# Celebrandil/CudaSift

Hardware: AMD Instinct MI355X
Metric: 1920x1080 SIFT frames/sec (higher is better)
Workload: dtype f32

## Files before the change

### cudasift_amd/csrc/kernels_dog.hip

```cpp
#include <stdlib.h>
#include <string.h>
#include <math.h>
#include "common.hpp"
#include "chain.hpp"

#define WAVES_PER_BLOCK 4
#define OUT_LANES 62

struct ItemCoord { int frame, strip, seg; bool valid; };

__device__ __forceinline__ ItemCoord decode_item(const StripGeom &g)
{
  const unsigned lb = (g.noremap & 1) ? blockIdx.x : xcd_remap(blockIdx.x, gridDim.x);
  const int wave = __builtin_amdgcn_readfirstlane((int)(threadIdx.x >> 6));
  const long long item = (long long)lb * WAVES_PER_BLOCK + wave;
  const long long nitems = (long long)g.nframes * g.nstrips * g.nsegs;
  ItemCoord c;
  c.valid = item < nitems;
  if (g.noremap & 2) {
    c.strip = (int)(item % g.nstrips);
    const long long r = item / g.nstrips;
    c.seg = (int)(r % g.nsegs);
    c.frame = (int)(r / g.nsegs);
  } else {
// ... 878 lines not shown
    if (threadIdx.x == 0) STAMP_MAX(14);
    if (threadIdx.x == 0 && lb + 1 == gridDim.x) STAMP_MAX(16);
    if (threadIdx.x == 0 && lb == (unsigned)nchain) STAMP_MAX(17);
#endif
    if (lb < (unsigned)nchain) {
      const int tiles = C.tiles_x * C.tiles_y;
#if SCAN_RING
      float *chain_lds = reinterpret_cast<float *>(&s_win[0][0]);
#else
      float *chain_lds = s_chain_lds;
#endif
      scaledown_chain_block(const_cast<float *>(scratch), C, k5, (int)(lb % tiles), (int)(lb / tiles), chain_lds);
      asm volatile("s_waitcnt vmcnt(0)" ::: "memory");
      __builtin_amdgcn_fence(__ATOMIC_RELEASE, "workgroup");
      __syncthreads();
      STAMP_MAX(9);
      if (threadIdx.x == 0) {
        unsigned *spare = counters + (size_t)G.nframes * CNT_STRIDE;
        const unsigned sub = lb & 15u, members = ((unsigned)nchain - sub + 15u) / 16u;
        if (atomicAdd(&spare[64 + 32 * sub], 1u) == members - 1u) {
          const unsigned nsub = (unsigned)nchain < 16u ? (unsigned)nchain : 16u;
          if (atomicAdd(&spare[32], 1u) == nsub - 1u && G.wait_ticks != 0u) {
            __hip_atomic_fetch_or(&spare[0], 0x80000000u, __ATOMIC_RELAXED, __HIP_MEMORY_SCOPE_AGENT);
            STAMP_MAX(18);
          }
        }
      }
      STAMP_MAX(19);
      return;
    }
    lb -= (unsigned)nchain;
    if (G.wait_lev < G.nlev && (long long)lb * WAVES_PER_BLOCK + (WAVES_PER_BLOCK - 1) >= G.o[G.wait_lev].item_begin) {
      STAMP_MAX(15);
      __shared__ unsigned s_chain_ok;
      if (threadIdx.x == 0) {
        const unsigned long long t0 = wall_clock64();
        unsigned ok = 1u;
        while ((__hip_atomic_fetch_add(&counters[(size_t)G.nframes * CNT_STRIDE], 1u, __ATOMIC_RELAXED, __HIP_MEMORY_SCOPE_AGENT) &
                0x80000000u) == 0u) {
          if (wall_clock64() - t0 > (unsigned long long)G.wait_ticks) { ok = 0u; break; }
          __builtin_amdgcn_s_sleep(8);
        }
        if (!ok) atomicAdd(&counters[CNT_CHAINTMO], 1u);
        s_chain_ok = ok;
      }
      __syncthreads();
      STAMP_MAX(13);
      __builtin_amdgcn_fence(__ATOMIC_ACQUIRE, "workgroup");
      chain_failed = s_chain_ok == 0u;
    }
  }
  long long item = (long long)lb * WAVES_PER_BLOCK + wave;
  const bool valid = item < G.total_items && !chain_failed;
  __shared__ unsigned s_cq[WAVES_PER_BLOCK][CQ_CAP];
  unsigned qn = 0;
  unsigned *cnt = nullptr, *list = nullptr;
  unsigned cand_cap = 0;
  int octave = 0;
  bool stamp_coarse = false;
  (void)stamp_coarse;
  if (valid) {
    int lev = 0;
    for (int k = 1; k < G.nlev; k++)
      if (item >= G.o[k].item_begin) lev = k;
    lev = __builtin_amdgcn_readfirstlane(lev);
    stamp_coarse = lev >= G.wait_lev;
    const ScanOct &L = G.o[lev];
    item -= L.item_begin;
    const int seg = (int)(item % L.nsegs);
    const long long r = item / L.nsegs;
    const int strip = (int)(r % L.nstrips);
    const int frame = (int)(r / L.nstrips);
    if (lane < NUM_SCAN_PAIRS * 5) s_taps[wave][lane] = scan_pair_tap(taps.t[L.octave], lane);
    wave_lds_fence();
    const int q = strip * (OUT_LANES - 2) + lane - 2;
    const int y0 = seg * L.seg_rows;
    cnt = counters + (size_t)frame * CNT_STRIDE;
    list = cand + (size_t)frame * G.cand_stride + L.cand_off;
    cand_cap = L.cand_cap;
    octave = L.octave;
#if SCAN_TAPS_REG
    const RegTaps tsrc(s_taps[wave]);
#else
    const LdsTaps tsrc{s_taps[wave]};
#endif
#if SCAN_RING
    scan_strip_ring<FAST>(scratch + (long long)frame * G.frame_stride + L.img_off, L.w, L.h, L.p, q, lane, y0,
                          min(y0 + L.seg_rows, L.h), tsrc, thresh, cnt, list, cand_cap, octave, FAST != 0,
                          &s_win[wave][lane], s_cq[wave], qn, xch);
#else
    scan_strip<FAST>(scratch + (long long)frame * G.frame_stride + L.img_off, L.w, L.h, L.p, q, lane, y0,
                     min(y0 + L.seg_rows, L.h), tsrc, thresh, cnt, list, cand_cap, octave, FAST != 0,
                     s_cq[wave], qn, xch);
#endif
  }
#if SCAN_STAMPS
  if (CHAIN && valid) { if (stamp_coarse) STAMP_MAX(12); else STAMP_MAX(11); }
#endif
  scan_queue_finish(s_cq[wave], qn, valid ? cnt + CNT_CAND + octave : nullptr, cnt, list, cand_cap);
}

struct RefineParams {
  int width, height, pitch, nframes;
  float edge_limit, factor, lowest_scale, subsampling, thresh;
  float scmul[NUM_SCALES];
  int octave, max_pts;
  unsigned cand_cap;
};

__device__ __forceinline__ void dog_patch(const float *img, int w, int h, int pitch, const float (&tk)[4][5],
                                          int x, int y, float (&d)[3][3][3])
{
  int xo[11];
#pragma unroll
  for (int cx = 0; cx < 11; cx++) xo[cx] = clampi(x + cx - 5, 0, w - 1);
  float prev[3][3];
#pragma unroll
  for (int bs = 0; bs < 4; bs++) {
    const float k0 = tk[bs][0], k1 = tk[bs][1], k2 = tk[bs][2], k3 = tk[bs][3], k4 = tk[bs][4];
    float vres[3][11];
#pragma unroll
    for (int cx = 0; cx < 11; cx++) {
      const float *col = img + xo[cx];
      float r[11];
#pragma unroll
      for (int j = 0; j < 11; j++) r[j] = col[(size_t)clampi(y + j - 5, 0, h - 1) * pitch];
#pragma unroll
      for (int dy = 0; dy < 3; dy++)
        vres[dy][cx] = conv9(k0, k1, k2, k3, k4, r[dy + 4], r[dy + 3] + r[dy + 5], r[dy + 2] + r[dy + 6],
                             r[dy + 1] + r[dy + 7], r[dy + 0] + r[dy + 8]);
    }
#pragma unroll
    for (int dy = 0; dy < 3; dy++)
#pragma unroll
      for (int dx = 0; dx < 3; dx++) {
        const float *v = &vres[dy][dx];
        const float cur = conv9(k0, k1, k2, k3, k4, v[4], v[3] + v[5], v[2] + v[6], v[1] + v[7], v[0] + v[8]);
        if (bs > 0) d[bs - 1][dy][dx] = cur - prev[dy][dx];
        prev[dy][dx] = cur;
      }
  }
}

__device__ __forceinline__ float det_exp2(float x)
{
  const bool tiny = x < -125.0f;
  x = x > 126.0f ? 126.0f : x;
  x = tiny ? 0.0f : x;
  const float n = rintf(x);
  const float r = x - n;
  float p = __builtin_fmaf(1.535336188319500e-4f, r, 1.339887440266574e-3f);
  p = __builtin_fmaf(p, r, 9.618437357674640e-3f);
  p = __builtin_fmaf(p, r, 5.550332471162809e-2f);
  p = __builtin_fmaf(p, r, 2.402264791363012e-1f);
  p = __builtin_fmaf(p, r, 6.931472028550421e-1f);
  p = __builtin_fmaf(p, r, 1.0f);
  const float sc = __builtin_bit_cast(float, ((int)n + 127) << 23);
  return tiny ? 0.0f : p * sc;
}

struct Refined { float xpos, ypos, scale, sharpness, edgeness; };
__device__ __forceinline__ bool refine_math(const float (&d)[3][3][3], int x, int y, int s, float thresh,
                                            float edge_limit, float factor, float lowest_scale,
                                            const float (&scmul)[NUM_SCALES], Refined &out, bool *extremum = nullptr)
{
  const float val = d[1][1][1];
  if (extremum) *extremum = false;
  {
    float minv = INFINITY, maxv = -INFINITY;
#pragma unroll
    for (int p = 0; p < 3; p++)
#pragma unroll
      for (int dy = 0; dy < 3; dy++)
#pragma unroll
        for (int dx = 0; dx < 3; dx++)
          if (!(p == 1 && dy == 1 && dx == 1)) {
            minv = fminf(minv, d[p][dy][dx]);
            maxv = fmaxf(maxv, d[p][dy][dx]);
          }
    if (!((val < fminf(-thresh, minv)) || (val > fmaxf(thresh, maxv)))) return false;
    if (extremum) *extremum = true;
  }
  const float dxx = 2.0f * val - d[1][1][0] - d[1][1][2];
  const float dyy = 2.0f * val - d[1][0][1] - d[1][2][1];
  const float dxy = 0.25f * (d[1][2][2] + d[1][0][0] - d[1][0][2] - d[1][2][0]);
  const float tra = dxx + dyy;
  const float det = dxx * dyy - dxy * dxy;
  if (!(tra * tra < edge_limit * det)) return false;
  const float edge = (tra * tra) / det;
  const float dx = 0.5f * (d[1][1][2] - d[1][1][0]);
  const float dy = 0.5f * (d[1][2][1] - d[1][0][1]);
  const float ds = 0.5f * (d[0][1][1] - d[2][1][1]);
  const float dss = 2.0f * val - d[2][1][1] - d[0][1][1];
  const float dxs = 0.25f * (d[2][1][2] + d[0][1][0] - d[0][1][2] - d[2][1][0]);
  const float dys = 0.25f * (d[2][2][1] + d[0][0][1] - d[2][0][1] - d[0][2][1]);
  const float idxx = dyy * dss - dys * dys;
  const float idxy = dys * dxs - dxy * dss;
  const float idxs = dxy * dys - dyy * dxs;
  const float idet = 1.0f / (idxx * dxx + idxy * dxy + idxs * dxs);
  const float idyy = dxx * dss - dxs * dxs;
  const float idys = dxy * dxs - dxx * dys;
  const float idss = dxx * dyy - dxy * dxy;
  float pdx = idet * (idxx * dx + idxy * dy + idxs * ds);
  float pdy = idet * (idxy * dx + idyy * dy + idys * ds);
  float pds = idet * (idxs * dx + idys * dy + idss * ds);
  if (pdx < -0.5f || pdx > 0.5f || pdy < -0.5f || pdy > 0.5f || pds < -0.5f || pds > 0.5f) {
    pdx = dx / dxx;
    pdy = dy / dyy;
    pds = ds / dss;
  }
  const float dval = 0.5f * (dx * pdx + dy * pdy + ds * pds);
  float scm = scmul[0];
#pragma unroll
  for (int j = 1; j < NUM_SCALES; j++) scm = (s == j) ? scmul[j] : scm;
  const float sc = scm * det_exp2(pds * factor);
  if (!(sc >= lowest_scale)) return false;
  out.xpos = x + pdx;
  out.ypos = y + pdy;
  out.scale = sc;
  out.sharpness = val + dval;
  out.edgeness = edge;
  return true;
}

__device__ __forceinline__ void dog_from_base(const float *img, int w, int h, int pitch, const LaplaceTaps &taps,
                                              int x, int y, int s, float (&d)[3][3][3])
{
  float tk[4][5];
#pragma unroll
  for (int bs = 0; bs < 4; bs++)
#pragma unroll
    for (int j = 0; j < 5; j++) {
      float t = taps.k[bs][j];
#pragma unroll
      for (int ss = 1; ss < NUM_SCALES; ss++) t = (s == ss) ? taps.k[ss + bs][j] : t;
      tk[bs][j] = t;
    }
  dog_patch(img, w, h, pitch, tk, x, y, d);
}

template <bool FROM_BASE>
__global__ __launch_bounds__(64) void refine_kernel(const float *__restrict__ src, long long src_frame_stride,
                                                    LaplaceTaps taps, RefineParams P,
                                                    unsigned *__restrict__ counters,
                                                    const unsigned *__restrict__ cand, SiftPointD *__restrict__ pts)
{
  const int frame = blockIdx.y;
  unsigned *cnt = counters + (size_t)frame * CNT_STRIDE;
  const unsigned *list = cand + (size_t)frame * P.cand_cap;
  SiftPointD *out = pts + (size_t)frame * P.max_pts;
  const float *img = src + (long long)frame * src_frame_stride;
  const int o = P.octave;
  if (blockIdx.x == 0 && threadIdx.x == 0) {
    const unsigned start = cnt[2 * o - 1];
    atomicMax(&cnt[2 * o + 0], start);
    atomicMax(&cnt[2 * o + 1], start);
  }
  const unsigned ncand = min(cnt[CNT_CAND + o], P.cand_cap);
  const size_t plane = (size_t)P.height * P.pitch;
  for (unsigned ci = blockIdx.x * blockDim.x + threadIdx.x; ci < ncand; ci += gridDim.x * blockDim.x) {
    const unsigned code = list[ci];
    if (code == 0xffffffffu) continue;
    const int x = code & 0x3fff, y = (code >> 14) & 0x3fff, s = code >> 28;
    float d[3][3][3];
    if (FROM_BASE) {
      dog_from_base(img, P.width, P.height, P.pitch, taps, x, y, s, d);
    } else {
#pragma unroll
      for (int p = 0; p < 3; p++)
#pragma unroll
        for (int dy = 0; dy < 3; dy++)
#pragma unroll
          for (int dx = 0; dx < 3; dx++)
            d[p][dy][dx] = img[(size_t)(s + p) * plane + (size_t)(y + dy - 1) * P.pitch + (x + dx - 1)];
    }
    Refined r;
    if (!refine_math(d, x, y, s, P.thresh, P.edge_limit, P.factor, P.lowest_scale, P.scmul, r)) continue;
    atomicMax(&cnt[2 * o + 0], cnt[2 * o - 1]);
    const unsigned idx = atomicAdd(&cnt[2 * o + 0], 1u);
    if (idx >= (unsigned)P.max_pts) { atomicAdd(&cnt[CNT_PTOVF], 1u); continue; }
    SiftPointD *p = &out[idx];
    p->xpos = r.xpos;
    p->ypos = r.ypos;
    p->scale = r.scale;
    p->sharpness = r.sharpness;
    p->edgeness = r.edgeness;
    p->subsampling = P.subsampling;
  }
}

#define REFCAP_W 30
#define REFCAP_H 8
#define REFCAP_WORDS 8
struct RefineAllParams {
  float thresh, edge_limit, factor;
  float scmul[NUM_SCALES];
  int max_pts;
  unsigned cand_stride;
  unsigned cap_words;
  unsigned cap_limit;
  unsigned cap_off[MISIFT_MAX_OCTAVES + 1];
  int cap_tx[MISIFT_MAX_OCTAVES + 1], cap_ty[MISIFT_MAX_OCTAVES + 1];
};
template <int CTRL>
__device__ __forceinline__ float row_dpp(float v)
{
  return __builtin_bit_cast(float, __builtin_amdgcn_mov_dpp(__builtin_bit_cast(int, v), CTRL, 0xf, 0xf, true));
}
#define ROW_SHR(n) (0x110 + (n))
#define ROW_SHL(n) (0x100 + (n))

__global__ __launch_bounds__(256) void refine_all_kernel(const float *__restrict__ scratch, PyramidInfo P,
                                                         AllTaps taps, RefineAllParams R,
                                                         unsigned *__restrict__ counters,
                                                         const unsigned *__restrict__ cand,
                                                         Detection *__restrict__ det, unsigned *__restrict__ capcnt)
{
  const int frame = blockIdx.y;
  unsigned *cnt = counters + (size_t)frame * CNT_STRIDE;
  Detection *fdet = det + (size_t)frame * MISIFT_MAX_OCTAVES * R.max_pts;
  const int lane = threadIdx.x & 63, c = lane & 15;
  const unsigned group = (blockIdx.x * 4u + (threadIdx.x >> 6)) * 4u + (unsigned)(lane >> 4);
  const unsigned ngroups = gridDim.x * 16u;
  unsigned ncand[MISIFT_MAX_OCTAVES + 1];
  unsigned total = 0;
#pragma unroll
  for (int k = 1; k <= MISIFT_MAX_OCTAVES; k++) {
    ncand[k] = k <= P.noct ? __builtin_amdgcn_readfirstlane(min(cnt[CNT_CAND + k], P.o[k].cand_cap)) : 0u;
    total += ncand[k];
  }
  __shared__ unsigned s_n[MISIFT_MAX_OCTAVES + 1], s_base[MISIFT_MAX_OCTAVES + 1];
  if (threadIdx.x <= MISIFT_MAX_OCTAVES) s_n[threadIdx.x] = 0;
  __syncthreads();
  const unsigned rounds = (total + ngroups - 1) / ngroups;
  for (unsigned it = 0; it < rounds; it++) {
    const unsigned fi = it * ngroups + group;
    const bool live = fi < total;
    int o = P.noct;
    unsigned ci = live ? fi : 0u;
    bool found = false;
#pragma unroll
    for (int k = MISIFT_MAX_OCTAVES; k >= 1; k--) {
      if (!found && k <= P.noct) {
        if (ci < ncand[k]) { o = k; found = true; }
        else ci -= ncand[k];
      }
    }
    const int lw = P.o[o].w, lh = P.o[o].h, lp = P.o[o].p;
    const float *img = scratch + (long long)frame * P.frame_stride + P.o[o].img_off;
    const unsigned code = live ? cand[(size_t)frame * R.cand_stride + P.o[o].cand_off + ci] : 0u;
    const int x = code & 0x3fff, y = (code >> 14) & 0x3fff, s = code >> 28;
    const float *col = img + clampi(x + min(c, 10) - 5, 0, lw - 1);
    float r[11];
#pragma unroll
    for (int j = 0; j < 11; j++) r[j] = col[(size_t)clampi(y + j - 5, 0, lh - 1) * lp];
    float ps[3][4];
#pragma unroll
    for (int dy = 0; dy < 3; dy++)
#pragma unroll
      for (int k = 1; k <= 4; k++) ps[dy][k - 1] = r[dy + 4 - k] + r[dy + 4 + k];
    float d[3][3];
    float prev[3];
#pragma unroll
    for (int bs = 0; bs < 4; bs++) {
      const float *tk = taps.t[o].k[s + bs];
      const float k0 = tk[0], k1 = tk[1], k2 = tk[2], k3 = tk[3], k4 = tk[4];
#pragma unroll
      for (int dy = 0; dy < 3; dy++) {
        const float v = conv9(k0, k1, k2, k3, k4, r[dy + 4], ps[dy][0], ps[dy][1], ps[dy][2], ps[dy][3]);
        const float cur = conv9(k0, k1, k2, k3, k4, v,
                                row_dpp<ROW_SHR(1)>(v) + row_dpp<ROW_SHL(1)>(v),
                                row_dpp<ROW_SHR(2)>(v) + row_dpp<ROW_SHL(2)>(v),
                                row_dpp<ROW_SHR(3)>(v) + row_dpp<ROW_SHL(3)>(v),
                                row_dpp<ROW_SHR(4)>(v) + row_dpp<ROW_SHL(4)>(v));
        if (bs > 0) d[bs - 1][dy] = cur - prev[dy];
        prev[dy] = cur;
      }
    }
    float dd[3][3][3];
#pragma unroll
    for (int p = 0; p < 3; p++)
#pragma unroll
      for (int dy = 0; dy < 3; dy++) {
        dd[p][dy][0] = row_dpp<ROW_SHR(1)>(d[p][dy]);
        dd[p][dy][1] = d[p][dy];
        dd[p][dy][2] = row_dpp<ROW_SHL(1)>(d[p][dy]);
      }
    Refined rr;
    bool extremum = false;
    const bool ok = live && c == 5 &&
                    refine_math(dd, x, y, s, R.thresh, R.edge_limit, R.factor, P.o[o].lowest_scale, R.scmul, rr, &extremum);
    if (R.cap_words && live && c == 5 && extremum) {
      const unsigned idx = R.cap_off[o] + ((unsigned)s * R.cap_ty[o] + (unsigned)(y / REFCAP_H)) * R.cap_tx[o] + (unsigned)(x / REFCAP_W);
      const unsigned sh = 8u * (idx & 3u);
      const unsigned old = atomicAdd(&capcnt[(size_t)frame * R.cap_words + (idx >> 2)], 1u << sh);
      if (((old >> sh) & 0xffu) == R.cap_limit) atomicAdd(&cnt[CNT_CANDOVF], 1u);
    }
    unsigned rank = 0;
    if (ok) rank = atomicAdd(&s_n[o], 1u);
    __syncthreads();
    if (threadIdx.x >= 1 && threadIdx.x <= MISIFT_MAX_OCTAVES) {
      const unsigned n = s_n[threadIdx.x];
      if (n) {
        s_base[threadIdx.x] = atomicAdd(&cnt[CNT_DET + threadIdx.x], n);
        s_n[threadIdx.x] = 0;
      }
    }
    __syncthreads();
    if (!ok) continue;
    const unsigned idx = s_base[o] + rank;
    if (idx >= (unsigned)R.max_pts) { atomicAdd(&cnt[CNT_PTOVF], 1u); continue; }
    Detection *pd = &fdet[(size_t)(o - 1) * R.max_pts + idx];
    pd->xpos = rr.xpos;
    pd->ypos = rr.ypos;
    pd->scale = rr.scale;
    pd->sharpness = rr.sharpness;
    pd->edgeness = rr.edgeness;
  }
}

static inline bool is_aligned16(const void *p, int pitch) { return (((uintptr_t)p) & 15) == 0 && (pitch & 3) == 0; }

static inline dim3 grid_for(const StripGeom &g)
{
  const long long nitems = (long long)g.nframes * g.nstrips * g.nsegs;
  return dim3((unsigned)((nitems + WAVES_PER_BLOCK - 1) / WAVES_PER_BLOCK));
}

int launch_laplace(misift_ctx *ctx, const float *base, const StripGeom &g, float *dog,
                   long long dog_frame_stride, const LaplaceTaps &taps)
{
  const int al = is_aligned16(base, g.pitch) && is_aligned16(dog, g.pitch) && (g.frame_stride & 3) == 0 &&
                 (dog_frame_stride & 3) == 0;
  LaunchScope ls(ctx, "laplace");
  if (al && (g.width & 3) == 0)
    hipLaunchKernelGGL(laplace_kernel<true>, grid_for(g), dim3(256), 0, ctx->stream, base, g, dog, dog_frame_stride,
                       taps, al);
  else
    hipLaunchKernelGGL(laplace_kernel<false>, grid_for(g), dim3(256), 0, ctx->stream, base, g, dog,
                       dog_frame_stride, taps, al);
  return ls.finish();
}

int launch_detect(misift_ctx *ctx, const float *dog, const StripGeom &g, long long dog_frame_stride,
                  float thresh, int octave)
{
  const int al = is_aligned16(dog, g.pitch) && (dog_frame_stride & 3) == 0;
  LaunchScope ls(ctx, "detect");
  hipLaunchKernelGGL(detect_kernel, grid_for(g), dim3(256), 0, ctx->stream, dog, g, dog_frame_stride, thresh,
                     octave, ctx->d_counters, ctx->d_cand, (unsigned)ctx->cand_cap, al);
  return ls.finish();
}

__device__ __forceinline__ void refcap_locate(unsigned code, int tiles_x, int tiles_y, size_t *word0, unsigned *bit)
{
  const int x = code & 0x3fff, y = (code >> 14) & 0x3fff, s = code >> 28;
  const int tx = x / REFCAP_W, ty = y / REFCAP_H;
  *word0 = (((size_t)s * tiles_y + ty) * tiles_x + tx) * REFCAP_WORDS;
  *bit = (unsigned)((x - tx * REFCAP_W) * REFCAP_H + (y - ty * REFCAP_H));
}
__global__ __launch_bounds__(256) void refcap_mark_kernel(const unsigned *__restrict__ counters, const unsigned *__restrict__ cand,
                                                          unsigned cand_cap, int octave, int tiles_x, int tiles_y,
                                                          unsigned *__restrict__ mask, size_t mask_words_per_frame)
{
  const int frame = blockIdx.y;
  const unsigned n = min(counters[(size_t)frame * CNT_STRIDE + CNT_CAND + octave], cand_cap);
  const unsigned *list = cand + (size_t)frame * cand_cap;
  unsigned *m = mask + (size_t)frame * mask_words_per_frame;
  for (unsigned i = blockIdx.x * blockDim.x + threadIdx.x; i < n; i += gridDim.x * blockDim.x) {
    size_t w0; unsigned bit;
    refcap_locate(list[i], tiles_x, tiles_y, &w0, &bit);
    atomicOr(&m[w0 + (bit >> 5)], 1u << (bit & 31u));
  }
}
__global__ __launch_bounds__(256) void refcap_drop_kernel(const unsigned *__restrict__ counters, unsigned *__restrict__ cand,
                                                          unsigned cand_cap, int octave, int tiles_x, int tiles_y,
                                                          const unsigned *__restrict__ mask, size_t mask_words_per_frame)
{
  const int frame = blockIdx.y;
  const unsigned n = min(counters[(size_t)frame * CNT_STRIDE + CNT_CAND + octave], cand_cap);
  unsigned *list = cand + (size_t)frame * cand_cap;
  const unsigned *m = mask + (size_t)frame * mask_words_per_frame;
  for (unsigned i = blockIdx.x * blockDim.x + threadIdx.x; i < n; i += gridDim.x * blockDim.x) {
    size_t w0; unsigned bit;
    refcap_locate(list[i], tiles_x, tiles_y, &w0, &bit);
    unsigned rank = 0;
    for (unsigned w = 0; w < (bit >> 5); w++) rank += __popc(m[w0 + w]);
    rank += __popc(m[w0 + (bit >> 5)] & ((1u << (bit & 31u)) - 1u));
    if (rank >= 32u) list[i] = 0xffffffffu;
  }
}

int launch_refcap(misift_ctx *ctx, int w, int h, int nframes, int octave)
{
  const int tiles_x = (w + REFCAP_W - 1) / REFCAP_W, tiles_y = (h + REFCAP_H - 1) / REFCAP_H;
  const size_t words = (size_t)NUM_SCALES * tiles_x * tiles_y * REFCAP_WORDS;
  if (sizeof(unsigned) * words * nframes > ctx->refcap_bytes) {
    if (ctx->d_refcap) { HIP_TRY(hipStreamSynchronize(ctx->stream)); HIP_TRY(misift_dev_free(ctx->d_refcap)); }
    ctx->d_refcap = nullptr; ctx->refcap_bytes = 0;
    HIP_TRY(misift_dev_alloc((void **)&ctx->d_refcap, sizeof(unsigned) * words * nframes, "refcap_masks"));
    ctx->refcap_bytes = sizeof(unsigned) * words * nframes;
  }
  HIP_TRY(hipMemsetAsync(ctx->d_refcap, 0, sizeof(unsigned) * words * nframes, ctx->stream));
  LaunchScope ls(ctx, "refcap");
  hipLaunchKernelGGL(refcap_mark_kernel, dim3(64, nframes), dim3(256), 0, ctx->stream, ctx->d_counters, ctx->d_cand,
                     (unsigned)ctx->cand_cap, octave, tiles_x, tiles_y, ctx->d_refcap, words);
  hipLaunchKernelGGL(refcap_drop_kernel, dim3(64, nframes), dim3(256), 0, ctx->stream, ctx->d_counters, ctx->d_cand,
                     (unsigned)ctx->cand_cap, octave, tiles_x, tiles_y, ctx->d_refcap, words);
  return ls.finish();
}

int launch_dog_scan(misift_ctx *ctx, const float *base, const StripGeom &g, const LaplaceTaps &taps,
                      float thresh, int octave)
{
  const int al0 = is_aligned16(base, g.pitch) && (g.frame_stride & 3) == 0;
  LaunchScope ls(ctx, "dog_scan");
  if (al0 && (g.width & 3) == 0)
    hipLaunchKernelGGL((dog_scan_kernel<true, 2>), grid_for(g), dim3(256), 0, ctx->stream, base, g, taps, thresh,
                       octave, ctx->d_counters, ctx->d_cand, (unsigned)ctx->cand_cap, al0);
  else
    hipLaunchKernelGGL((dog_scan_kernel<false, 2>), grid_for(g), dim3(256), 0, ctx->stream, base, g, taps, thresh,
                       octave, ctx->d_counters, ctx->d_cand, (unsigned)ctx->cand_cap, al0);
  return ls.finish();
}

int launch_refine(misift_ctx *ctx, const float *dog, long long dog_frame_stride, const float *base,
                  long long base_frame_stride, const LaplaceTaps *taps, int w, int h, int pitch, int nframes,
                  float thresh, float edge_limit, float factor, float lowest_scale, float subsampling, int octave,
                  SiftPointD *pts, int max_pts)
{
  RefineParams P;
  P.width = w; P.height = h; P.pitch = pitch; P.nframes = nframes;
  P.edge_limit = edge_limit; P.factor = factor; P.lowest_scale = lowest_scale; P.subsampling = subsampling;
  P.thresh = thresh;
  for (int s = 0; s < NUM_SCALES; s++) P.scmul[s] = powf(2.0f, (float)s / NUM_SCALES);
  P.octave = octave; P.max_pts = max_pts; P.cand_cap = (unsigned)ctx->cand_cap;
  LaplaceTaps t;
  if (taps) t = *taps; else memset(&t, 0, sizeof(t));
  const dim3 grid(128, nframes);
  LaunchScope ls(ctx, "refine");
  if (dog)
    hipLaunchKernelGGL(refine_kernel<false>, grid, dim3(64), 0, ctx->stream, dog, dog_frame_stride, t, P,
                       ctx->d_counters, ctx->d_cand, pts);
  else
    hipLaunchKernelGGL(refine_kernel<true>, grid, dim3(64), 0, ctx->stream, base, base_frame_stride, t, P,
                       ctx->d_counters, ctx->d_cand, pts);
  return ls.finish();
}

static AllTaps pack_taps(const LaplaceTaps *taps, int noct)
{
  AllTaps a;
  memset(&a, 0, sizeof(a));
  for (int o = 1; o <= noct; o++) a.t[o] = taps[o];
  return a;
}

struct CapLayout { unsigned words; unsigned off[MISIFT_MAX_OCTAVES + 1]; int tx[MISIFT_MAX_OCTAVES + 1], ty[MISIFT_MAX_OCTAVES + 1]; };
static CapLayout cap_layout(const PyramidInfo &P)
{
  CapLayout L;
  memset(&L, 0, sizeof(L));
  unsigned n = 0;
  for (int o = 1; o <= P.noct; o++) {
    L.off[o] = n;
    L.tx[o] = (P.o[o].w + REFCAP_W - 1) / REFCAP_W;
    L.ty[o] = (P.o[o].h + REFCAP_H - 1) / REFCAP_H;
    n += (unsigned)NUM_SCALES * L.tx[o] * L.ty[o];
  }
  L.words = (n + 3u) / 4u;
  return L;
}
static int ensure_capcnt(misift_ctx *ctx, const PyramidInfo &P, const CapLayout &L)
{
  const size_t bytes = sizeof(unsigned) * (size_t)L.words * P.nframes;
  if (bytes > ctx->capcnt_bytes) {
    if (ctx->d_capcnt) { HIP_TRY(hipStreamSynchronize(ctx->stream)); HIP_TRY(misift_dev_free(ctx->d_capcnt)); }
    ctx->d_capcnt = nullptr; ctx->capcnt_bytes = 0;
    HIP_TRY(misift_dev_alloc((void **)&ctx->d_capcnt, bytes, "refcap_counts"));
    ctx->capcnt_bytes = bytes;
    ctx->alloc_gen++;
  }
  return MISIFT_OK;
}

int launch_dog_scan_all(misift_ctx *ctx, const float *scratch, const PyramidInfo &P, const LaplaceTaps *taps,
                        float thresh, int lev_begin, int lev_end, const ChainGeom *chain, const float *k5)
{
  ScanAllGeom G;
  memset(&G, 0, sizeof(G));
  G.nlev = lev_end - lev_begin; G.nframes = P.nframes; G.frame_stride = P.frame_stride;
  bool fast = (is_aligned16(scratch, 4) && (P.frame_stride & 3) == 0), ragged = false;
  long long items = 0;
  unsigned cand_stride = 0;
  for (int o = 1; o <= P.noct; o++) cand_stride += P.o[o].cand_cap;
  G.cand_stride = cand_stride;
  for (int lev = lev_begin; lev < lev_end; lev++) {
    const int o = P.noct - lev;
    const OctaveInfo &L = P.o[o];
    ScanOct &S = G.o[lev - lev_begin];
    S.w = L.w; S.h = L.h; S.p = L.p; S.octave = o; S.img_off = L.img_off;
    S.cand_off = L.cand_off; S.cand_cap = L.cand_cap;
    const int nquads = (L.w + 3) / 4;
    S.nstrips = (nquads + (OUT_LANES - 2) - 1) / (OUT_LANES - 2);
    if (S.nstrips < 1) S.nstrips = 1;
    const long long target = (long long)ctx->num_cus * ctx->scan_waves_per_cu;
    long long want = (target + (long long)P.nframes * S.nstrips - 1) / ((long long)P.nframes * S.nstrips);
    if (want < 1) want = 1;
    int seg = (int)((L.h + want - 1) / want);
#if SCAN_RING || SCAN_UNROLL9
    if (P.nframes <= ctx->small_frames) {
      const int floor_rows = (chain && lev - lev_begin >= 2) ? ctx->scan_rows_small_coarse : ctx->scan_rows_small;
      if (seg < floor_rows) seg = floor_rows;
      if (seg > RING_ROWS) seg = (seg + RING_ROWS - 1) / RING_ROWS * RING_ROWS;
    } else {
      seg = (seg + RING_ROWS - 1) / RING_ROWS * RING_ROWS;
      if (seg < 2 * RING_ROWS) seg = 2 * RING_ROWS;
    }
    if (seg > 14 * RING_ROWS) seg = 14 * RING_ROWS;
#else
    seg = (seg + 7) / 8 * 8;
    if (seg < 16) seg = 16;
    if (seg > 128) seg = 128;
#endif
    S.seg_rows = seg;
    S.nsegs = (L.h + seg - 1) / seg;
    S.item_begin = items;
    items += (long long)P.nframes * S.nstrips * S.nsegs;
    if ((L.p & 3) != 0 || (L.img_off & 3) != 0) fast = false;
    if ((L.w & 3) != 0) ragged = true;
  }
  G.total_items = items;
  if (ctx->opt.reference_cap && lev_begin == 0) {
    const CapLayout L = cap_layout(P);
    const int rc = ensure_capcnt(ctx, P, L);
    if (rc) return rc;
    G.cap_clear = ctx->d_capcnt;
    G.cap_clear_words = L.words * (unsigned)P.nframes;
  }
  const AllTaps at = pack_taps(taps, P.noct);
  ChainGeom C;
  Taps5 t5;
  memset(&C, 0, sizeof(C));
  memset(&t5, 0, sizeof(t5));
  int nchain = 0;
  if (chain) {
    C = *chain;
    for (int j = 0; j < 5; j++) t5.k[j] = k5[j];
    nchain = C.tiles_x * C.tiles_y * P.nframes;
    G.wait_lev = 0;
    G.wait_ticks = ctx->chain_wait_ticks;
    for (int k = 0; k < G.nlev; k++)
      if (G.o[k].img_off == C.lv[0].off) G.wait_lev = k + 1;
  }
  const dim3 grid((unsigned)((items + WAVES_PER_BLOCK - 1) / WAVES_PER_BLOCK) + (unsigned)nchain);
  LaunchScope ls(ctx, "dog_scan");
#define SCAN_LAUNCH(F, CH) hipLaunchKernelGGL((dog_scan_all_kernel<F, CH>), grid, dim3(256), (size_t)ctx->lds_pad_scan, ctx->stream, scratch, G, at, \
                                              thresh, ctx->d_counters, ctx->d_cand, C, t5, nchain)
  if (chain) {
    if (fast && !ragged) SCAN_LAUNCH(1, true);
    else if (fast) SCAN_LAUNCH(2, true);
    else SCAN_LAUNCH(0, true);
  } else {
    if (fast && !ragged) SCAN_LAUNCH(1, false);
    else if (fast) SCAN_LAUNCH(2, false);
    else SCAN_LAUNCH(0, false);
  }
#undef SCAN_LAUNCH
  return ls.finish();
}

int launch_refine_all(misift_ctx *ctx, const float *scratch, const PyramidInfo &P, const LaplaceTaps *taps,
                      float thresh, float edge_limit, float factor, int max_pts)
{
  RefineAllParams R;
  R.thresh = thresh; R.edge_limit = edge_limit; R.factor = factor; R.max_pts = max_pts;
  for (int s = 0; s < NUM_SCALES; s++) R.scmul[s] = powf(2.0f, (float)s / NUM_SCALES);
  unsigned cand_stride = 0;
  for (int o = 1; o <= P.noct; o++) cand_stride += P.o[o].cand_cap;
  R.cand_stride = cand_stride;
  R.cap_words = 0;
  if (ctx->opt.reference_cap) {
    const CapLayout L = cap_layout(P);
    const int rc = ensure_capcnt(ctx, P, L);
    if (rc) return rc;
    for (int o = 1; o <= P.noct; o++) { R.cap_off[o] = L.off[o]; R.cap_tx[o] = L.tx[o]; R.cap_ty[o] = L.ty[o]; }
    R.cap_words = L.words;
    R.cap_limit = (unsigned)ctx->refcap_limit;
  }
  const AllTaps at = pack_taps(taps, P.noct);
  LaunchScope ls(ctx, "refine");
  const int gx = P.nframes <= ctx->small_frames ? 1024 / P.nframes : 64;
  hipLaunchKernelGGL(refine_all_kernel, dim3(gx, P.nframes), dim3(256), 0, ctx->stream, scratch, P, at, R,
                     ctx->d_counters, ctx->d_cand, ctx->d_det, ctx->d_capcnt);
  return ls.finish();
}

__global__ void test_exp2_kernel(const float *__restrict__ x, float *__restrict__ out, int n)
{
  const int i = blockIdx.x * blockDim.x + threadIdx.x;
  if (i < n) out[i] = det_exp2(x[i]);
}
int launch_test_exp2(misift_ctx *ctx, const float *x, float *out, int n)
{
  hipLaunchKernelGGL(test_exp2_kernel, dim3((n + 255) / 256), dim3(256), 0, ctx->stream, x, out, n);
  HIP_TRY(hipGetLastError());
  return MISIFT_OK;
}
```

Baseline: 61740.

## Batch refine rounds through LDS so all 64 lanes run refine_math

The refine kernel now runs the separable Gaussian blur per candidate in batches of up to 16 rounds. Vertical-pass results go through LDS to a horizontal pass computed by 9 lanes, and the 3x3x3 DoG neighbourhood is stored in LDS. After each batch, every lane of the wave loads one candidate's neighbourhood and runs refine_math, instead of only lane 5 of each 16-lane group, which raises lane utilisation of the expensive refinement math. The candidate-to-octave lookup becomes a branchless prefix compare, and the grid width for large frame counts now scales with the frame count. The change adds LDS traffic, wave-level fences and more LDS per block, which may lower occupancy.

```diff
diff --git a/cudasift_amd/csrc/kernels_dog.hip b/cudasift_amd/csrc/kernels_dog.hip
--- a/cudasift_amd/csrc/kernels_dog.hip
+++ b/cudasift_amd/csrc/kernels_dog.hip
@@ -1204,13 +1204,8 @@
   unsigned cap_off[MISIFT_MAX_OCTAVES + 1];
   int cap_tx[MISIFT_MAX_OCTAVES + 1], cap_ty[MISIFT_MAX_OCTAVES + 1];
 };
-template <int CTRL>
-__device__ __forceinline__ float row_dpp(float v)
-{
-  return __builtin_bit_cast(float, __builtin_amdgcn_mov_dpp(__builtin_bit_cast(int, v), CTRL, 0xf, 0xf, true));
-}
-#define ROW_SHR(n) (0x110 + (n))
-#define ROW_SHL(n) (0x100 + (n))
+#define REFINE_BATCH 16
+#define REFINE_VCAND 144
 
 __global__ __launch_bounds__(256) void refine_all_kernel(const float *__restrict__ scratch, PyramidInfo P,
                                                          AllTaps taps, RefineAllParams R,
@@ -1221,78 +1216,100 @@
   const int frame = blockIdx.y;
   unsigned *cnt = counters + (size_t)frame * CNT_STRIDE;
   Detection *fdet = det + (size_t)frame * MISIFT_MAX_OCTAVES * R.max_pts;
-  const int lane = threadIdx.x & 63, c = lane & 15;
-  const unsigned group = (blockIdx.x * 4u + (threadIdx.x >> 6)) * 4u + (unsigned)(lane >> 4);
+  const int lane = threadIdx.x & 63, wave = threadIdx.x >> 6, c = lane & 15, grp = lane >> 4;
+  const unsigned group0 = (blockIdx.x * 4u + (unsigned)wave) * 4u;
   const unsigned ngroups = gridDim.x * 16u;
-  unsigned ncand[MISIFT_MAX_OCTAVES + 1];
+  unsigned first[MISIFT_MAX_OCTAVES + 1];
   unsigned total = 0;
 #pragma unroll
-  for (int k = 1; k <= MISIFT_MAX_OCTAVES; k++) {
-    ncand[k] = k <= P.noct ? __builtin_amdgcn_readfirstlane(min(cnt[CNT_CAND + k], P.o[k].cand_cap)) : 0u;
-    total += ncand[k];
+  for (int k = MISIFT_MAX_OCTAVES; k >= 1; k--) {
+    first[k] = k <= P.noct ? total : ~0u;
+    total += k <= P.noct ? __builtin_amdgcn_readfirstlane(min(cnt[CNT_CAND + k], P.o[k].cand_cap)) : 0u;
   }
   __shared__ unsigned s_n[MISIFT_MAX_OCTAVES + 1], s_base[MISIFT_MAX_OCTAVES + 1];
+  __shared__ float s_v[4][4 * REFINE_VCAND];
+  __shared__ float s_d[4][64 * 27];
   if (threadIdx.x <= MISIFT_MAX_OCTAVES) s_n[threadIdx.x] = 0;
   __syncthreads();
+  auto locate = [&](unsigned fi, int &o, unsigned &code) -> bool {
+    const bool live = fi < total;
+    const unsigned f = live ? fi : 0u;
+    unsigned fo = 0;
+    o = P.noct;
+#pragma unroll
+    for (int k = MISIFT_MAX_OCTAVES - 1; k >= 1; k--) {
+      const bool in = f >= first[k];
+      o = in ? k : o;
+      fo = in ? first[k] : fo;
+    }
+    code = live ? cand[(size_t)frame * R.cand_stride + P.o[o].cand_off + (f - fo)] : 0u;
+    return live;
+  };
+  float *vcol = s_v[wave] + grp * REFINE_VCAND + min(c, 10);
+  const float *vrow = s_v[wave] + grp * REFINE_VCAND + (c / 3) * 11 + c % 3;
+  float *dslot = s_d[wave] + grp * 27 + c;
   const unsigned rounds = (total + ngroups - 1) / ngroups;
-  for (unsigned it = 0; it < rounds; it++) {
-    const unsigned fi = it * ngroups + group;
-    const bool live = fi < total;
-    int o = P.noct;
-    unsigned ci = live ? fi : 0u;
-    bool found = false;
-#pragma unroll
-    for (int k = MISIFT_MAX_OCTAVES; k >= 1; k--) {
-      if (!found && k <= P.noct) {
-        if (ci < ncand[k]) { o = k; found = true; }
-        else ci -= ncand[k];
+  const unsigned nbatch = (rounds + REFINE_BATCH - 1) / REFINE_BATCH;
+  for (unsigned b = 0; b < nbatch; b++) {
+    const unsigned nr = min(rounds - b * REFINE_BATCH, (unsigned)REFINE_BATCH);
+    for (unsigned rb = 0; rb < nr; rb++) {
+      int o;
+      unsigned code;
+      locate((b * REFINE_BATCH + rb) * ngroups + group0 + (unsigned)grp, o, code);
+      const int lw = P.o[o].w, lh = P.o[o].h, lp = P.o[o].p;
+      const float *img = scratch + (long long)frame * P.frame_stride + P.o[o].img_off;
+      const int x = code & 0x3fff, y = (code >> 14) & 0x3fff, s = code >> 28;
+      const float *col = img + clampi(x + min(c, 10) - 5, 0, lw - 1);
+      float r[11];
+#pragma unroll
+      for (int j = 0; j < 11; j++) r[j] = col[(size_t)clampi(y + j - 5, 0, lh - 1) * lp];
+      float ps[3][4];
+#pragma unroll
+      for (int dy = 0; dy < 3; dy++)
+#pragma unroll
+        for (int k = 1; k <= 4; k++) ps[dy][k - 1] = r[dy + 4 - k] + r[dy + 4 + k];
+      float tk[4][5];
+#pragma unroll
+      for (int bs = 0; bs < 4; bs++) {
+#pragma unroll
+        for (int j = 0; j < 5; j++) tk[bs][j] = taps.t[o].k[s + bs][j];
+#pragma unroll
+        for (int dy = 0; dy < 3; dy++) {
+          const float v = conv9(tk[bs][0], tk[bs][1], tk[bs][2], tk[bs][3], tk[bs][4], r[dy + 4], ps[dy][0], ps[dy][1],
+                                ps[dy][2], ps[dy][3]);
+          if (c < 11) vcol[(bs * 3 + dy) * 11] = v;
+        }
       }
-    }
-    const int lw = P.o[o].w, lh = P.o[o].h, lp = P.o[o].p;
-    const float *img = scratch + (long long)frame * P.frame_stride + P.o[o].img_off;
-    const unsigned code = live ? cand[(size_t)frame * R.cand_stride + P.o[o].cand_off + ci] : 0u;
+      wave_lds_fence();
+      if (c < 9) {
+        float prev = 0.0f;
+#pragma unroll
+        for (int bs = 0; bs < 4; bs++) {
+          const float *v = vrow + bs * 33;
+          const float cur = conv9(tk[bs][0], tk[bs][1], tk[bs][2], tk[bs][3], tk[bs][4], v[4], v[3] + v[5], v[2] + v[6],
+                                  v[1] + v[7], v[0] + v[8]);
+          if (bs > 0) dslot[rb * 108 + (bs - 1) * 9] = cur - prev;
+          prev = cur;
+        }
+      }
+      wave_lds_fence();
+    }
+    int o;
+    unsigned code;
+    const bool live = locate((b * REFINE_BATCH + (unsigned)(lane >> 2)) * ngroups + group0 + (unsigned)(lane & 3), o, code);
     const int x = code & 0x3fff, y = (code >> 14) & 0x3fff, s = code >> 28;
-    const float *col = img + clampi(x + min(c, 10) - 5, 0, lw - 1);
-    float r[11];
-#pragma unroll
-    for (int j = 0; j < 11; j++) r[j] = col[(size_t)clampi(y + j - 5, 0, lh - 1) * lp];
-    float ps[3][4];
-#pragma unroll
-    for (int dy = 0; dy < 3; dy++)
-#pragma unroll
-      for (int k = 1; k <= 4; k++) ps[dy][k - 1] = r[dy + 4 - k] + r[dy + 4 + k];
-    float d[3][3];
-    float prev[3];
-#pragma unroll
-    for (int bs = 0; bs < 4; bs++) {
-      const float *tk = taps.t[o].k[s + bs];
-      const float k0 = tk[0], k1 = tk[1], k2 = tk[2], k3 = tk[3], k4 = tk[4];
-#pragma unroll
-      for (int dy = 0; dy < 3; dy++) {
-        const float v = conv9(k0, k1, k2, k3, k4, r[dy + 4], ps[dy][0], ps[dy][1], ps[dy][2], ps[dy][3]);
-        const float cur = conv9(k0, k1, k2, k3, k4, v,
-                                row_dpp<ROW_SHR(1)>(v) + row_dpp<ROW_SHL(1)>(v),
-                                row_dpp<ROW_SHR(2)>(v) + row_dpp<ROW_SHL(2)>(v),
-                                row_dpp<ROW_SHR(3)>(v) + row_dpp<ROW_SHL(3)>(v),
-                                row_dpp<ROW_SHR(4)>(v) + row_dpp<ROW_SHL(4)>(v));
-        if (bs > 0) d[bs - 1][dy] = cur - prev[dy];
-        prev[dy] = cur;
-      }
-    }
     float dd[3][3][3];
 #pragma unroll
     for (int p = 0; p < 3; p++)
 #pragma unroll
-      for (int dy = 0; dy < 3; dy++) {
-        dd[p][dy][0] = row_dpp<ROW_SHR(1)>(d[p][dy]);
-        dd[p][dy][1] = d[p][dy];
-        dd[p][dy][2] = row_dpp<ROW_SHL(1)>(d[p][dy]);
-      }
+      for (int dy = 0; dy < 3; dy++)
+#pragma unroll
+        for (int dx = 0; dx < 3; dx++) dd[p][dy][dx] = s_d[wave][lane * 27 + p * 9 + dy * 3 + dx];
     Refined rr;
     bool extremum = false;
-    const bool ok = live && c == 5 &&
+    const bool ok = live &&
                     refine_math(dd, x, y, s, R.thresh, R.edge_limit, R.factor, P.o[o].lowest_scale, R.scmul, rr, &extremum);
-    if (R.cap_words && live && c == 5 && extremum) {
+    if (R.cap_words && live && extremum) {
       const unsigned idx = R.cap_off[o] + ((unsigned)s * R.cap_ty[o] + (unsigned)(y / REFCAP_H)) * R.cap_tx[o] + (unsigned)(x / REFCAP_W);
       const unsigned sh = 8u * (idx & 3u);
       const unsigned old = atomicAdd(&capcnt[(size_t)frame * R.cap_words + (idx >> 2)], 1u << sh);
@@ -1309,15 +1326,19 @@
       }
     }
     __syncthreads();
-    if (!ok) continue;
-    const unsigned idx = s_base[o] + rank;
-    if (idx >= (unsigned)R.max_pts) { atomicAdd(&cnt[CNT_PTOVF], 1u); continue; }
-    Detection *pd = &fdet[(size_t)(o - 1) * R.max_pts + idx];
-    pd->xpos = rr.xpos;
-    pd->ypos = rr.ypos;
-    pd->scale = rr.scale;
-    pd->sharpness = rr.sharpness;
-    pd->edgeness = rr.edgeness;
+    if (ok) {
+      const unsigned idx = s_base[o] + rank;
+      if (idx >= (unsigned)R.max_pts) {
+        atomicAdd(&cnt[CNT_PTOVF], 1u);
+      } else {
+        Detection *pd = &fdet[(size_t)(o - 1) * R.max_pts + idx];
+        pd->xpos = rr.xpos;
+        pd->ypos = rr.ypos;
+        pd->scale = rr.scale;
+        pd->sharpness = rr.sharpness;
+        pd->edgeness = rr.edgeness;
+      }
+    }
   }
 }
 
@@ -1592,7 +1613,7 @@
   }
   const AllTaps at = pack_taps(taps, P.noct);
   LaunchScope ls(ctx, "refine");
-  const int gx = P.nframes <= ctx->small_frames ? 1024 / P.nframes : 64;
+  const int gx = P.nframes <= ctx->small_frames ? 1024 / P.nframes : std::min(64, std::max(16, 1024 / P.nframes));
   hipLaunchKernelGGL(refine_all_kernel, dim3(gx, P.nframes), dim3(256), 0, ctx->stream, scratch, P, at, R,
                      ctx->d_counters, ctx->d_cand, ctx->d_det, ctx->d_capcnt);
   return ls.finish();
```

New measurement: 62100 (median of 4 runs). No clear change (+0.6%).
